# kabachuha/sd-webui-text2video

Hardware: NVIDIA H100
Metric: denoised frames/sec (UNet+VAE) ModelScope 24fx256^2 50-step (higher is better)
Workload: dtype f16 (fp32 accumulate / norms / softmax)

## Files before the change

### sd-webui-text2video_b200/csrc/elementwise.cu

```cuda
#include "common.cuh"
#include "kernels.cuh"

#include <math_constants.h>

namespace t2v {

namespace {

inline int grid_for(long long n, int threads, int cap = 132 * 16) {
    long long b = (n + threads - 1) / threads;
    if (b > cap) b = cap;
    if (b < 1) b = 1;
    return static_cast<int>(b);
}
#define GRID_STRIDE(i, n) \
    for (long long i = blockIdx.x * static_cast<long long>(blockDim.x) + threadIdx.x; i < (n); \
         i += static_cast<long long>(gridDim.x) * blockDim.x)

__global__ void ingest_kernel(const void* x, int x_is_f32, __half* tok, long long ld, int cpad, int C, int F, int h, int w,
                              long long frame0, long long nframes, float scale) {
    const long long P = static_cast<long long>(h) * w;
    const long long rows = nframes * P;
    GRID_STRIDE(i, rows * cpad) {
        const long long r = i / cpad;
        const int c = static_cast<int>(i - r * cpad);
        float v = 0.f;
        if (c < C) {
            const long long p = r % P;
            const long long bf = frame0 + r / P;
            const int f = static_cast<int>(bf % F);
            const int b = static_cast<int>(bf / F);
            const long long src = ((static_cast<long long>(b) * C + c) * F + f) * P + p;
            v = x_is_f32 ? reinterpret_cast<const float*>(x)[src] : __half2float(reinterpret_cast<const __half*>(x)[src]);
            v *= scale;
        }
        tok[r * ld + c] = __float2half_rn(v);
    }
}

__global__ void egress_kernel(const __half* tok, long long ld, void* out, int out_is_f32, int B, int C, int F, int h,
                              int w) {
    const long long P = static_cast<long long>(h) * w;
    const long long n = static_cast<long long>(B) * C * F * P;
    GRID_STRIDE(i, n) {
        const long long p = i % P;
        long long t = i / P;
        const int f = static_cast<int>(t % F);
        t /= F;
        const int c = static_cast<int>(t % C);
        const int b = static_cast<int>(t / C);
        const __half v = tok[((static_cast<long long>(b) * F + f) * P + p) * ld + c];
        if (out_is_f32) reinterpret_cast<float*>(out)[i] = __half2float(v);
        else reinterpret_cast<__half*>(out)[i] = v;
    }
}

__global__ void upsample2x_kernel(const uint4* x, uint4* y, long long nframes, int h, int w, int C8) {
    const int H = 2 * h, W = 2 * w;
    const long long n = nframes * H * W * C8;
    GRID_STRIDE(i, n) {
        const int c = static_cast<int>(i % C8);
        long long t = i / C8;
        const int X = static_cast<int>(t % W);
        t /= W;
        const int Y = static_cast<int>(t % H);
        const long long f = t / H;
        y[i] = __ldg(x + ((f * h + (Y >> 1)) * w + (X >> 1)) * C8 + c);
    }
}

__global__ void im2col_s2_kernel(const uint4* x, uint4* col, long long nframes, int h, int w, int C8, int pad_lo) {
    const int ho = pad_lo ? (h + 1) / 2 : h / 2, wo = pad_lo ? (w + 1) / 2 : w / 2;
    const long long n = nframes * ho * wo * 9 * C8;
    GRID_STRIDE(i, n) {
        const int c = static_cast<int>(i % C8);
        long long t = i / C8;
        const int tap = static_cast<int>(t % 9);
        t /= 9;
        const int xo = static_cast<int>(t % wo);
        t /= wo;
        const int yo = static_cast<int>(t % ho);
        const long long f = t / ho;
        const int yi = 2 * yo + tap / 3 - pad_lo;
        const int xi = 2 * xo + tap % 3 - pad_lo;
        uint4 v = make_uint4(0, 0, 0, 0);
        if (yi >= 0 && yi < h && xi >= 0 && xi < w) v = __ldg(x + ((f * h + yi) * w + xi) * C8 + c);
        col[i] = v;
    }
}

__global__ void concat_kernel(const __half* a, long long lda, int Ca8, const __half* b, long long ldb, int Cb8,
                              __half* out, long long ldo, long long rows) {
    const int T8 = Ca8 + Cb8;
    GRID_STRIDE(i, rows * T8) {
        const long long r = i / T8;
        const int c = static_cast<int>(i - r * T8);
        uint4 v;
        if (c < Ca8) v = __ldg(reinterpret_cast<const uint4*>(a + r * lda) + c);
        else v = __ldg(reinterpret_cast<const uint4*>(b + r * ldb) + (c - Ca8));
        reinterpret_cast<uint4*>(out + r * ldo)[c] = v;
    }
}

__global__ void time_sinusoid_kernel(const float* t, __half* out, int B, int dim) {
    const int half_dim = dim / 2;
    GRID_STRIDE(i, static_cast<long long>(B) * dim) {
        const int b = static_cast<int>(i / dim);
        const int j = static_cast<int>(i % dim);
        float v = 0.f;
        if (j < 2 * half_dim) {
            const int k = j < half_dim ? j : j - half_dim;
            const float freq = powf(10000.0f, -(static_cast<float>(k) / static_cast<float>(half_dim)));
            const float s = t[b] * freq;
            v = j < half_dim ? cosf(s) : sinf(s);
        }
        out[i] = __float2half_rn(v);
    }
}

__global__ void __launch_bounds__(256) small_linear_kernel(const __half* x, long long ldx, const __half* W,
                                                           const __half* bias, const __half* addend, __half* y,
                                                           long long ldy, int B, int N, int K, int silu_in) {
    const int lane = threadIdx.x & 31;
    const int n = blockIdx.x * (blockDim.x >> 5) + (threadIdx.x >> 5);
    if (n >= N) return;
    const __half* wr = W + static_cast<long long>(n) * K;
    for (int b = 0; b < B; ++b) {
        float acc = 0.f;
        for (int k = lane * 8; k < K; k += 256) {
            const uint4 wv = __ldg(reinterpret_cast<const uint4*>(wr + k));
            const uint4 xv = __ldg(reinterpret_cast<const uint4*>(x + b * ldx + k));
            const __half* wh = reinterpret_cast<const __half*>(&wv);
            const __half* xh = reinterpret_cast<const __half*>(&xv);
#pragma unroll
            for (int e = 0; e < 8; ++e) {
                float xe = __half2float(xh[e]);
                if (silu_in) xe = __half2float(__float2half_rn(xe / (1.0f + __expf(-xe))));
                acc += xe * __half2float(wh[e]);
            }
        }
#pragma unroll
        for (int o = 16; o > 0; o >>= 1) acc += __shfl_xor_sync(0xffffffffu, acc, o);
        if (lane == 0) {
            if (bias) acc += __half2float(bias[n]);
            float r = __half2float(__float2half_rn(acc));
            if (addend) r += __half2float(addend[n]);
            y[b * ldy + n] = __float2half_rn(r);
        }
    }
}

__global__ void __launch_bounds__(256) softmax_rows_kernel(const __half* x, __half* y, long long rows, int cols,
                                                           float scale) {
    const int lane = threadIdx.x & 31;
    const long long row = blockIdx.x * static_cast<long long>(blockDim.x >> 5) + (threadIdx.x >> 5);
    if (row >= rows) return;
    const __half* xr = x + row * cols;
    float m = -CUDART_INF_F;
    for (int c = lane; c < cols; c += 32) m = fmaxf(m, __half2float(__float2half_rn(__half2float(xr[c]) * scale)));
#pragma unroll
    for (int o = 16; o > 0; o >>= 1) m = fmaxf(m, __shfl_xor_sync(0xffffffffu, m, o));
    float s = 0.f;
    for (int c = lane; c < cols; c += 32) s += __expf(__half2float(__float2half_rn(__half2float(xr[c]) * scale)) - m);
#pragma unroll
    for (int o = 16; o > 0; o >>= 1) s += __shfl_xor_sync(0xffffffffu, s, o);
    const float inv = 1.0f / s;
    __half* yr = y + row * cols;
    for (int c = lane; c < cols; c += 32)
        yr[c] = __float2half_rn(__expf(__half2float(__float2half_rn(__half2float(xr[c]) * scale)) - m) * inv);
}

__global__ void transpose_kernel(const __half* x, __half* y, int R, int C) {
    __shared__ __half tile[32][34];
    const long long base = static_cast<long long>(blockIdx.z) * R * C;
    const int c0 = blockIdx.x * 32, r0 = blockIdx.y * 32;
    for (int j = threadIdx.y; j < 32; j += 8) {
        const int r = r0 + j, c = c0 + threadIdx.x;
        if (r < R && c < C) tile[j][threadIdx.x] = x[base + static_cast<long long>(r) * C + c];
    }
    __syncthreads();
    for (int j = threadIdx.y; j < 32; j += 8) {
        const int c = c0 + j, r = r0 + threadIdx.x;
        if (r < R && c < C) y[base + static_cast<long long>(c) * R + r] = tile[threadIdx.x][j];
    }
}

__global__ void frames_to_u8_kernel(const __half* tok, long long ld, uint8_t* out, long long pixels) {
    GRID_STRIDE(i, pixels * 3) {
        const long long p = i / 3;
        const int c = static_cast<int>(i - p * 3);
        float v = __half2float(tok[p * ld + c]);
        v = __fadd_rn(__fmul_rn(v, 0.5f), 0.5f);
        v = fminf(fmaxf(v, 0.f), 1.f);
        out[i] = static_cast<uint8_t>(__fmul_rn(v, 255.0f));
    }
}

__global__ void pixel_unshuffle_kernel(const void* x, int x_is_f32, __half* tok, int N, int Cc, int H, int W) {
    const int h8 = H / 8, w8 = W / 8;
    const int groups = Cc * 8;
    const long long n = static_cast<long long>(N) * h8 * w8 * groups;
    GRID_STRIDE(i, n) {
        const int g = static_cast<int>(i % groups);
        long long t = i / groups;
        const int xo = static_cast<int>(t % w8);
        t /= w8;
        const int yo = static_cast<int>(t % h8);
        const long long f = t / h8;
        const int c = g >> 3, ky = g & 7;
        const long long src = ((f * Cc + c) * H + (8 * yo + ky)) * static_cast<long long>(W) + 8 * xo;
        uint4 o;
        __half* oh = reinterpret_cast<__half*>(&o);
#pragma unroll
        for (int j = 0; j < 8; ++j)
            oh[j] = x_is_f32 ? __float2half_rn(reinterpret_cast<const float*>(x)[src + j]) : reinterpret_cast<const __half*>(x)[src + j];
        reinterpret_cast<uint4*>(tok)[i] = o;
    }
}

__global__ void relu_kernel(uint4* x, long long n8) {
    const __half2 z = __float2half2_rn(0.f);
    GRID_STRIDE(i, n8) {
        uint4 v = x[i];
        __half2* h = reinterpret_cast<__half2*>(&v);
#pragma unroll
        for (int k = 0; k < 4; ++k) h[k] = __hmax2_nan(h[k], z);
        x[i] = v;
    }
}

__global__ void avgpool2x2_kernel(const uint4* x, uint4* y, long long nframes, int h, int w, int C8) {
    const int ho = h / 2, wo = w / 2;
    GRID_STRIDE(i, nframes * ho * wo * C8) {
        const int c = static_cast<int>(i % C8);
        long long t = i / C8;
        const int xo = static_cast<int>(t % wo);
        t /= wo;
        const int yo = static_cast<int>(t % ho);
        const long long f = t / ho;
        float acc[8] = {0.f, 0.f, 0.f, 0.f, 0.f, 0.f, 0.f, 0.f};
#pragma unroll
        for (int tap = 0; tap < 4; ++tap) {
            const uint4 v = __ldg(x + ((f * h + 2 * yo + (tap >> 1)) * w + 2 * xo + (tap & 1)) * C8 + c);
            const __half2* hv = reinterpret_cast<const __half2*>(&v);
#pragma unroll
            for (int k = 0; k < 4; ++k) {
                const float2 a = __half22float2(hv[k]);
                acc[2 * k] += a.x;
                acc[2 * k + 1] += a.y;
            }
        }
        uint4 o;
        __half2* oh = reinterpret_cast<__half2*>(&o);
#pragma unroll
        for (int k = 0; k < 4; ++k) oh[k] = __floats2half2_rn(acc[2 * k] * 0.25f, acc[2 * k + 1] * 0.25f);
        y[i] = o;
    }
}

__global__ void feature_add_kernel(__half* x, long long ldx, const __half* f, int C8, long long rows, long long rows_per_sample,
                                   int f_samples) {
    GRID_STRIDE(i, rows * C8) {
        const long long r = i / C8;
        const int c = static_cast<int>(i - r * C8);
        const long long s = r / rows_per_sample;
        const long long fr = (s % f_samples) * rows_per_sample + (r - s * rows_per_sample);
        uint4* xp = reinterpret_cast<uint4*>(x + r * ldx) + c;
        uint4 a = *xp;
        const uint4 b = __ldg(reinterpret_cast<const uint4*>(f + fr * (static_cast<long long>(C8) * 8)) + c);
        __half2* ah = reinterpret_cast<__half2*>(&a);
        const __half2* bh = reinterpret_cast<const __half2*>(&b);
#pragma unroll
        for (int k = 0; k < 4; ++k) {
            const float2 u = __half22float2(ah[k]), v = __half22float2(bh[k]);
            ah[k] = __floats2half2_rn(u.x + v.x, u.y + v.y);
        }
        *xp = a;
    }
}

__global__ void frames_to_f32_kernel(const __half* tok, long long ld, float* out, int n, int H, int W) {
    const long long P = static_cast<long long>(H) * W;
    GRID_STRIDE(i, static_cast<long long>(n) * 3 * P) {
        const long long p = i % P;
        const long long t = i / P;
        const int c = static_cast<int>(t % 3);
        const long long f = t / 3;
        out[i] = __half2float(tok[(f * P + p) * ld + c]);
    }
}

__global__ void pack_conv_kernel(const void* src, int src_is_f32, __half* dst, int Cout, int Cin, int taps, int n_alloc,
// ... 201 lines not shown
        out[i] = __dadd_rn(__dmul_rn(a, __dsub_rn(1.0, m)), __dmul_rn(noise[i], m));
        if (mask != nullptr) mask[i] = m;
    }
}

__global__ void q_sample_blend_kernel(QSampleBlendParams p) {
    const long long hw = static_cast<long long>(p.shape[3]) * p.shape[4];
    const long long n = static_cast<long long>(p.shape[0]) * p.shape[1] * p.shape[2] * hw;
    GRID_STRIDE(i, n) {
        const int x = static_cast<int>(i % p.shape[4]);
        long long r = i / p.shape[4];
        const int y = static_cast<int>(r % p.shape[3]);
        r /= p.shape[3];
        const int t = static_cast<int>(r % p.shape[2]);
        r /= p.shape[2];
        const int c = static_cast<int>(r % p.shape[1]);
        const int b = static_cast<int>(r / p.shape[1]);
        const int idx[5] = {b, c, t, y, x};
        long long ox = 0, on = 0, om = 0;
#pragma unroll
        for (int d = 0; d < 5; ++d) {
            ox += idx[d] * p.x0_stride[d];
            on += idx[d] * p.noise_stride[d];
            om += idx[d] * p.mask_stride[d];
        }
        const float known = __fadd_rn(__fmul_rn(p.a[b], p.x0[ox]), __fmul_rn(p.s[b], p.noise[on]));
        if (p.mask == nullptr) {
            p.out[i] = known;
        } else {
            const float m = p.mask[om];
            p.out[i] = __fadd_rn(__fmul_rn(known, m), __fmul_rn(__fsub_rn(1.0f, m), p.img[i]));
        }
    }
}

__global__ void lora_merge_kernel(__half* __restrict__ w, const __half* __restrict__ A, const __half* __restrict__ B, int out, int cols,
                                  int rank, float alpha, int temporal_mean) {
    const long long n = static_cast<long long>(out) * cols;
    const int a_cols = temporal_mean ? cols * 3 : cols;
    GRID_STRIDE(i, n) {
        const int o = static_cast<int>(i / cols);
        const int j = static_cast<int>(i - static_cast<long long>(o) * cols);
        float d;
        if (temporal_mean) {
            float sum = 0.f;
            for (int q = 0; q < 3; ++q) {
                float acc = 0.f;
                for (int r = 0; r < rank; ++r)
                    acc = fmaf(__half2float(B[static_cast<long long>(o) * rank + r]), __half2float(A[static_cast<long long>(r) * a_cols + j * 3 + q]), acc);
                sum += __half2float(__float2half_rn(acc));
            }
            d = __half2float(__float2half_rn(sum / 3.0f));
        } else {
            float acc = 0.f;
            for (int r = 0; r < rank; ++r)
                acc = fmaf(__half2float(B[static_cast<long long>(o) * rank + r]), __half2float(A[static_cast<long long>(r) * a_cols + j]), acc);
            d = __half2float(__float2half_rn(acc));
        }
        const float scaled = __half2float(__float2half_rn(d * alpha));
        w[i] = __float2half_rn(__half2float(w[i]) + scaled);
    }
}

__device__ __forceinline__ float widen(float v) { return v; }
__device__ __forceinline__ float widen(__half v) { return __half2float(v); }

template <class T>
__global__ void lora_apply_kernel(__half* __restrict__ w, const T* __restrict__ up, const T* __restrict__ down, int out, int cols,
                                  int rank, float alpha) {
    const long long n = static_cast<long long>(out) * cols;
    GRID_STRIDE(i, n) {
        const int o = static_cast<int>(i / cols);
        const int j = static_cast<int>(i - static_cast<long long>(o) * cols);
        float acc = 0.f;
        for (int r = 0; r < rank; ++r)
            acc = fmaf(widen(up[static_cast<long long>(o) * rank + r]), widen(down[static_cast<long long>(r) * cols + j]), acc);
        w[i] = __float2half_rn(__fadd_rn(__half2float(w[i]), __fmul_rn(alpha, acc)));
    }
}

inline int ok() { return launch_status("elementwise launch"); }

}

int ingest_latent(const void* x, int x_is_f32, __half* tok, long long ld, int cpad, int B, int C, int F, int h, int w,
                  float scale, cudaStream_t stream) {
    return ingest_latent_frames(x, x_is_f32, tok, ld, cpad, C, F, h, w, 0, static_cast<long long>(B) * F, scale, stream);
}
int ingest_latent_frames(const void* x, int x_is_f32, __half* tok, long long ld, int cpad, int C, int F, int h, int w,
                         long long frame0, long long nframes, float scale, cudaStream_t stream) {
    const long long n = nframes * h * w * cpad;
    ingest_kernel<<<grid_for(n, 256), 256, 0, stream>>>(x, x_is_f32, tok, ld, cpad, C, F, h, w, frame0, nframes, scale);
    return ok();
}
int egress_latent(const __half* tok, long long ld, void* out, int out_is_f32, int B, int C, int F, int h, int w,
                  cudaStream_t stream) {
    const long long n = static_cast<long long>(B) * C * F * h * w;
    egress_kernel<<<grid_for(n, 256), 256, 0, stream>>>(tok, ld, out, out_is_f32, B, C, F, h, w);
    return ok();
}
int upsample2x(const __half* x, __half* y, int nframes, int h, int w, int C, cudaStream_t stream) {
    if (C % 8) return -1;
    const long long n = static_cast<long long>(nframes) * 4 * h * w * (C / 8);
    upsample2x_kernel<<<grid_for(n, 256), 256, 0, stream>>>(reinterpret_cast<const uint4*>(x), reinterpret_cast<uint4*>(y),
                                                            nframes, h, w, C / 8);
    return ok();
}
int im2col_s2(const __half* x, __half* col, int nframes, int h, int w, int C, cudaStream_t stream, int pad_lo) {
    if (C % 8) return -1;
    const long long n = static_cast<long long>(nframes) * ((pad_lo ? (h + 1) / 2 : h / 2)) * ((pad_lo ? (w + 1) / 2 : w / 2)) * 9 * (C / 8);
    im2col_s2_kernel<<<grid_for(n, 256), 256, 0, stream>>>(reinterpret_cast<const uint4*>(x), reinterpret_cast<uint4*>(col),
                                                           nframes, h, w, C / 8, pad_lo);
    return ok();
}
int pixel_unshuffle_ingest(const void* x, int x_is_f32, __half* tok, int N, int Cc, int H, int W, cudaStream_t stream) {
    if (H % 8 || W % 8) return -1;
    const long long n = static_cast<long long>(N) * (H / 8) * (W / 8) * Cc * 8;
    pixel_unshuffle_kernel<<<grid_for(n, 256), 256, 0, stream>>>(x, x_is_f32, tok, N, Cc, H, W);
    return ok();
}
int relu_inplace(__half* x, long long rows, int C, cudaStream_t stream) {
    if (C % 8) return -1;
    const long long n8 = rows * (C / 8);
    relu_kernel<<<grid_for(n8, 256), 256, 0, stream>>>(reinterpret_cast<uint4*>(x), n8);
    return ok();
}
int avgpool2x2(const __half* x, __half* y, int nframes, int h, int w, int C, cudaStream_t stream) {
    if (C % 8) return -1;
    const long long n = static_cast<long long>(nframes) * (h / 2) * (w / 2) * (C / 8);
    avgpool2x2_kernel<<<grid_for(n, 256), 256, 0, stream>>>(reinterpret_cast<const uint4*>(x), reinterpret_cast<uint4*>(y),
                                                            nframes, h, w, C / 8);
    return ok();
}
int feature_add(__half* x, long long ldx, const __half* f, int C, long long rows, long long rows_per_sample, int f_samples,
                cudaStream_t stream) {
    if (C % 8 || ldx % 8 || rows_per_sample < 1 || f_samples < 1) return -1;
    const long long n = rows * (C / 8);
    feature_add_kernel<<<grid_for(n, 256), 256, 0, stream>>>(x, ldx, f, C / 8, rows, rows_per_sample, f_samples);
    return ok();
}
int concat_cols(const __half* a, long long lda, int Ca, const __half* b, long long ldb, int Cb, __half* out,
                long long ldo, long long rows, cudaStream_t stream) {
    if ((Ca % 8) || (Cb % 8) || (lda % 8) || (ldb % 8) || (ldo % 8)) return -1;
    const long long n = rows * ((Ca + Cb) / 8);
    concat_kernel<<<grid_for(n, 256), 256, 0, stream>>>(a, lda, Ca / 8, b, ldb, Cb / 8, out, ldo, rows);
    return ok();
}
int time_sinusoid(const float* t, __half* out, int B, int dim, cudaStream_t stream) {
    time_sinusoid_kernel<<<grid_for(static_cast<long long>(B) * dim, 256), 256, 0, stream>>>(t, out, B, dim);
    return ok();
}
int small_linear(const __half* x, long long ldx, const __half* W, const __half* bias, const __half* addend, __half* y,
                 long long ldy, int B, int N, int K, int silu_in, cudaStream_t stream) {
    if ((K % 8) || (ldx % 8)) return -1;
    small_linear_kernel<<<(N + 7) / 8, 256, 0, stream>>>(x, ldx, W, bias, addend, y, ldy, B, N, K, silu_in);
    return ok();
}
int softmax_rows(const __half* x, __half* y, long long rows, int cols, float scale, cudaStream_t stream) {
    softmax_rows_kernel<<<static_cast<unsigned int>((rows + 7) / 8), 256, 0, stream>>>(x, y, rows, cols, scale);
    return ok();
}
int transpose_batched(const __half* x, __half* y, int nb, int R, int C, cudaStream_t stream) {
    dim3 grid((C + 31) / 32, (R + 31) / 32, nb);
    transpose_kernel<<<grid, dim3(32, 8), 0, stream>>>(x, y, R, C);
    return ok();
}
int frames_to_u8(const __half* tok, long long ld, uint8_t* out, long long pixels, cudaStream_t stream) {
    frames_to_u8_kernel<<<grid_for(pixels * 3, 256), 256, 0, stream>>>(tok, ld, out, pixels);
    return ok();
}
int frames_to_f32_nchw(const __half* tok, long long ld, float* out, int n, int H, int W, cudaStream_t stream) {
    frames_to_f32_kernel<<<grid_for(static_cast<long long>(n) * 3 * H * W, 256), 256, 0, stream>>>(tok, ld, out, n, H, W);
    return ok();
}
int pack_conv_weight(const void* src, int src_is_f32, __half* dst, int Cout, int Cin, int taps, int n_alloc, int k_alloc,
                     cudaStream_t stream) {
    const long long n = static_cast<long long>(taps) * n_alloc * k_alloc;
    pack_conv_kernel<<<grid_for(n, 256), 256, 0, stream>>>(src, src_is_f32, dst, Cout, Cin, taps, n_alloc, k_alloc);
    return ok();
}
int pack_geglu_weight(const void* w, const void* b, int src_is_f32, __half* wdst, __half* bdst, int H, int K, int bn,
                      cudaStream_t stream) {
    if ((2 * H) % bn) return -1;
    pack_geglu_kernel<<<grid_for(static_cast<long long>(2) * H * K, 256), 256, 0, stream>>>(w, b, src_is_f32, wdst, bdst, H, K, bn);
    return ok();
}
int splitk_reduce(const float* part, int splits, long long split_stride, long long rows, int N, const __half* bias,
                  int bias_rows, long long bias_stride, const __half* residual, long long ldr, __half* out, long long ldo,
                  cudaStream_t stream) {
    if ((N & 7) || (ldo & 7) || (residual && (ldr & 7)) || (bias && (bias_stride & 7))) return -1;
    splitk_reduce_kernel<<<grid_for(rows * (N / 8), 256), 256, 0, stream>>>(part, splits, split_stride, rows, N / 8, bias,
                                                                            bias_rows, bias_stride, residual, ldr, out, ldo);
    return ok();
}
int fold_ln_into_linear(const __half* w, const __half* bias, const __half* gamma, const __half* beta, __half* wout,
                        float* colsum, float* bias32, int N, int K, cudaStream_t stream) {
    fold_ln_kernel<<<(N + 7) / 8, 256, 0, stream>>>(w, bias, gamma, beta, wout, colsum, bias32, N, K);
    return ok();
}
int convert_to_f16(const void* src, int src_is_f32, __half* dst, long long n, cudaStream_t stream) {
    convert_kernel<<<grid_for(n, 256), 256, 0, stream>>>(src, src_is_f32, dst, n);
    return ok();
}
int ddim_step(const DdimStepParams& p, cudaStream_t stream) {
    ddim_step_kernel<<<grid_for(p.n, 256), 256, 0, stream>>>(p);
    return ok();
}
int ddim_threshold_step(const DdimStepParams& p, int B, float percentile, float* s, void* ws, cudaStream_t stream) {
    if (percentile > 0.f) {
        ddim_x0_kernel<<<grid_for(p.n, 256), 256, 0, stream>>>(p);
        int rc = ok();
        if (rc != 0) return rc;
        if ((rc = abs_quantile(p.x_out, B, p.n / B, percentile, s, ws, stream)) != 0) return rc;
    }
    ddim_threshold_kernel<<<grid_for(p.n, 256), 256, 0, stream>>>(p, percentile > 0.f ? s : nullptr, p.n / B);
    return ok();
}
int lincomb(float* out, const float* const* src, const float* coef, int n_src, long long n, cudaStream_t stream) {
    if (n_src < 1 || n_src > 8) return -1;
    LincombArgs a;
    for (int i = 0; i < n_src; ++i) {
        a.src[i] = src[i];
        a.coef[i] = coef[i];
    }
    a.n_src = n_src;
    lincomb_kernel<<<grid_for(n, 256), 256, 0, stream>>>(out, a, n);
    return ok();
}
int lora_merge_weight(__half* w, const __half* A, const __half* B, int out, int cols, int rank, float alpha, int temporal_mean,
                      cudaStream_t stream) {
    const long long n = static_cast<long long>(out) * cols;
    lora_merge_kernel<<<grid_for(n, 256), 256, 0, stream>>>(w, A, B, out, cols, rank, alpha, temporal_mean);
    return ok();
}
int lora_apply_weight(__half* w, const void* up, const void* down, int dtype, int out, int cols, int rank, float alpha,
                      cudaStream_t stream) {
    const long long n = static_cast<long long>(out) * cols;
    if (dtype == 1)
        lora_apply_kernel<float><<<grid_for(n, 256), 256, 0, stream>>>(w, static_cast<const float*>(up),
                                                                       static_cast<const float*>(down), out, cols, rank, alpha);
    else
        lora_apply_kernel<__half><<<grid_for(n, 256), 256, 0, stream>>>(w, static_cast<const __half*>(up),
                                                                        static_cast<const __half*>(down), out, cols, rank, alpha);
    return ok();
}

int latent_blend(const float* img, int img_frames, const double* noise, const double* w, double* out, double* mask, int BC, int F,
                 long long hw, cudaStream_t stream) {
    const long long n = static_cast<long long>(BC) * F * hw;
    latent_blend_kernel<<<grid_for(n, 256), 256, 0, stream>>>(img, img_frames, noise, w, out, mask, n, F, hw);
    return ok();
}

int q_sample_blend(const QSampleBlendParams& p, cudaStream_t stream) {
    const long long n = static_cast<long long>(p.shape[0]) * p.shape[1] * p.shape[2] * p.shape[3] * p.shape[4];
    q_sample_blend_kernel<<<grid_for(n, 256), 256, 0, stream>>>(p);
    return ok();
}

int cfg_x0(const float* x, const void* eps_c, const void* eps_u, int eps_is_f32, float* x0, long long n, float g,
           float alpha, float sigma, int cfg_fp16, cudaStream_t stream) {
    cfg_x0_kernel<<<grid_for(n, 256), 256, 0, stream>>>(x, eps_c, eps_u, eps_is_f32, x0, n, g, alpha, sigma, cfg_fp16);
    return ok();
}

}
```

### sd-webui-text2video_b200/csrc/unet.cu

```cuda
#include "../../include/t2v_b200.h"
#include "runtime.cuh"

#include <algorithm>
#include <cmath>
#include <cstdlib>
#include <cstdio>
#include <cstring>
#include <memory>

namespace t2v {

namespace {

struct Blk {
    enum Kind { STEM, RES, ST, TT, DOWN, UP, STT } kind;
    std::string prefix;
    int cin = 0, cout = 0, heads = 0, inner = 0;
};

constexpr int kMaxFeat = 8;

struct IO {
    __half* x_tok;
    float* t;
// ... 180 lines not shown
                lin(p + ".proj_in", b.inner, b.cin);
                tblock(p + ".transformer_blocks.0", b.inner, c.context_dim);
                lin(p + ".proj_out", b.cin, b.inner);
                break;
            case Blk::TT:
                norm(p + ".norm", b.cin);
                P.expect(p + ".proj_in.weight", {b.inner, b.cin, 1});
                P.expect(p + ".proj_in.bias", {b.inner});
                tblock(p + ".transformer_blocks.0", b.inner, b.inner);
                P.expect(p + ".proj_out.weight", {b.cin, b.inner, 1});
                P.expect(p + ".proj_out.bias", {b.cin});
                break;
            case Blk::DOWN:
                P.expect(p + ".op.weight", {b.cout, b.cin, 3, 3});
                P.expect(p + ".op.bias", {b.cout});
                break;
            case Blk::UP:
                P.expect(p + ".conv.weight", {b.cout, b.cin, 3, 3});
                P.expect(p + ".conv.bias", {b.cout});
                break;
        }
    }
    norm("out.0", c.dim);
    P.expect("out.2.weight", {c.out_dim, c.dim, 3, 3});
    P.expect("out.2.bias", {c.out_dim});
}


void enumerate_vc(t2v_unet* u) {
    const t2v_unet_config& c = u->cfg;
    const int mc = c.dim, nm = c.n_mult;
    auto name = [](const char* base, int n, int k) {
        char buf[64];
        snprintf(buf, sizeof(buf), "%s.%d.%d", base, n, k);
        return std::string(buf);
    };
    u->ins.push_back({Blk{Blk::STEM, "input_blocks.0.0", c.in_dim, mc, 0, 0}});
    std::vector<int> chans{mc};
    int ch = mc;
    float scale = 1.0f;
    for (int level = 0; level < nm; ++level) {
        for (int j = 0; j < c.num_res_blocks; ++j) {
            const int n = static_cast<int>(u->ins.size());
            std::vector<Blk> blk;
            blk.push_back(Blk{Blk::RES, name("input_blocks", n, 0), ch, mc * c.dim_mult[level], 0, 0});
            ch = mc * c.dim_mult[level];
            if (in_scales(c, scale)) blk.push_back(Blk{Blk::STT, name("input_blocks", n, 1), ch, ch, c.num_heads, ch});
            u->ins.push_back(blk);
            chans.push_back(ch);
        }
        if (level != nm - 1) {
            const int n = static_cast<int>(u->ins.size());
            u->ins.push_back({Blk{Blk::DOWN, name("input_blocks", n, 0), ch, ch, 0, 0}});
            chans.push_back(ch);
            scale /= 2.0f;
        }
    }
    u->mid = {Blk{Blk::RES, "middle_block.0", ch, ch, 0, 0}, Blk{Blk::STT, "middle_block.1", ch, ch, c.num_heads, ch},
              Blk{Blk::RES, "middle_block.2", ch, ch, 0, 0}};
    for (int level = nm - 1; level >= 0; --level) {
        for (int i = 0; i < c.num_res_blocks + 1; ++i) {
            const int n = static_cast<int>(u->outs.size());
            const int ich = chans.back();
            chans.pop_back();
            std::vector<Blk> blk;
            blk.push_back(Blk{Blk::RES, name("output_blocks", n, 0), ch + ich, mc * c.dim_mult[level], 0, 0});
            ch = mc * c.dim_mult[level];
            if (in_scales(c, scale))
                blk.push_back(Blk{Blk::STT, name("output_blocks", n, static_cast<int>(blk.size())), ch, ch, c.num_heads, ch});
            if (level != 0 && i == c.num_res_blocks) {
                blk.push_back(Blk{Blk::UP, name("output_blocks", n, static_cast<int>(blk.size())), ch, ch, 0, 0});
                scale *= 2.0f;
            }
            u->outs.push_back(blk);
        }
    }
}

void expect_params_vc(t2v_unet* u) {
    ParamStore& P = u->params;
    const t2v_unet_config& c = u->cfg;
    const int E = c.dim * 4;
    auto lin = [&](const std::string& p, int o, int i, bool bias = true) {
        P.expect(p + ".weight", {o, i});
        if (bias) P.expect(p + ".bias", {o});
    };
    auto norm = [&](const std::string& p, int ch) {
        P.expect(p + ".weight", {ch});
        P.expect(p + ".bias", {ch});
    };
    auto conv = [&](const std::string& p, int o, int i, int k) {
        P.expect(p + ".weight", {o, i, 1, k, k});
        P.expect(p + ".bias", {o});
    };
    lin("time_embed.0", E, c.dim);
    lin("time_embed.2", E, E);
    std::vector<Blk> all;
    for (auto& b : u->ins) all.insert(all.end(), b.begin(), b.end());
    all.insert(all.end(), u->mid.begin(), u->mid.end());
    for (auto& b : u->outs) all.insert(all.end(), b.begin(), b.end());
    for (const Blk& b : all) {
        const std::string& p = b.prefix;
        switch (b.kind) {
            case Blk::STEM: conv(p, b.cout, b.cin, 3); break;
            case Blk::RES:
                norm(p + ".in_layers.0", b.cin);
                conv(p + ".in_layers.2", b.cout, b.cin, 3);
                lin(p + ".emb_layers.1", b.cout, E);
                norm(p + ".out_layers.0", b.cout);
                conv(p + ".out_layers.3", b.cout, b.cout, 3);
                if (b.cin != b.cout) conv(p + ".skip_connection", b.cout, b.cin, 1);
                break;
            case Blk::STT: {
                const int inner = b.inner, d = inner / b.heads;
                norm(p + ".norm", b.cin);
                conv(p + ".proj_in", inner, b.cin, 1);
                conv(p + ".proj_out", b.cin, inner, 1);
                const std::string t = p + ".transformer_blocks.0";
                const char* att[4] = {"attn1", "attn2", "attn1_tmp", "attn2_tmp"};
                for (int a = 0; a < 4; ++a) {
                    const std::string ap = t + "." + att[a];
                    const int kd = a == 1 ? c.context_dim : inner;
                    lin(ap + ".to_q", inner, inner, false);
                    lin(ap + ".to_k", inner, kd, false);
                    lin(ap + ".to_v", inner, kd, false);
                    lin(ap + ".to_out.0", inner, inner);
                    if (a >= 2) {
                        P.expect(ap + ".relative_position_k.embeddings_table", {2 * c.temporal_length + 1, d});
                        P.expect(ap + ".relative_position_v.embeddings_table", {2 * c.temporal_length + 1, d});
                    }
                }
                lin(t + ".ff.net.0.proj", inner * 8, inner);
                lin(t + ".ff.net.2", inner, inner * 4);
                for (int n = 1; n <= 5; ++n) norm(t + ".norm" + std::to_string(n), inner);
                break;
            }
            case Blk::DOWN: conv(p + ".op", b.cout, b.cin, 3); break;
            case Blk::UP: conv(p + ".conv", b.cout, b.cin, 3); break;
            default: break;
        }
    }
    norm("out.0", c.dim);
    conv("out.2", c.out_dim, c.dim, 3);
}

struct Ctx : NetCtx {
    t2v_unet* u;
    int B, F, h, w, L;
    int Bc;
    int Fl;
    int rank, nranks;
    char* slab;
    __half* emb;
    __half* ctx;
    Plan* plan;
};

int own_pixels(const Ctx& c, int hcur, int wcur) {
    if (c.nranks <= 1) return hcur * wcur;
    int pb[SHARD_MAX_RANKS + 1];
    shard_partition(hcur * wcur, c.nranks, pb);
    return pb[c.rank + 1] - pb[c.rank];
}

Tok exchange(Ctx& c, const Tok& x, bool to_ps, int hcur, int wcur) {
    const int P = hcur * wcur;
    const int np = own_pixels(c, hcur, wcur);
    const long long rows = to_ps ? static_cast<long long>(c.B) * c.F * np : static_cast<long long>(c.B) * c.Fl * P;
    Tok y = c.b->alloc(rows, x.C);
    PlanShard* ps = c.plan_shard;
    const int k = ps->n_xchg++;
    if (k >= SHARD_MAX_XCHG - 1) {
        set_error("frame-sharded plan: more than %d layout exchanges", SHARD_MAX_XCHG - 1);
        c.b->error = -31;
        return y;
    }
    if (!c.b->dry()) ps->dst_off[k] = reinterpret_cast<char*>(y.p) - c.slab;
    XchgParams xp;
    memset(&xp, 0, sizeof(xp));
    xp.slot = k;
    xp.to_ps = to_ps ? 1 : 0;
    xp.B = c.B; xp.F = c.F; xp.P = P; xp.C = x.C;
    xp.ld_src = x.ld; xp.ld_dst = y.ld;
    xp.src = x.p;
    for (int r = 0; r <= c.nranks; ++r) xp.fb[r] = ps->fb[r];
    shard_partition(P, c.nranks, xp.pb);
    const ShardPeers* peers = c.shard_peers;
    const int me = c.rank, nr = c.nranks, sms = c.b->sms();
    __half* own = y.p;
    char lab[96];
    snprintf(lab, sizeof(lab), "exchange %s rows=%lld C=%d", to_ps ? "FS->PS" : "PS->FS", rows, x.C);
    c.b->step([=](cudaStream_t s) {
        if (!ps->connected) return -40;
        XchgParams q = xp;
        q.peers = *peers;
        for (int r = 0; r < nr; ++r)
            q.dst[r] = r == me ? own : reinterpret_cast<__half*>(ps->peer_slab[r] + ps->peer_dst_off[r][k]);
        return shard_exchange(q, sms, s);
    }, 1, STEP_OTHER, 0.0, lab);
    return y;
}

void tap(Ctx& c, const std::string& name, const Tok& t, int h, int w) {
    if (c.u->taps_enabled && !c.b->dry()) c.plan->taps[name] = {t, {h, w}};
}

long long norm_rows(const Ctx& c, long long P) { return c.u->cfg.arch == 1 ? P * c.F : P; }


AttnParams attn_params(const Tok& o, int heads) {
    AttnParams a;
    memset(&a, 0, sizeof(a));
    a.o = o.p;
    a.heads = heads;
    a.head_dim = o.C / heads;
    a.scale = 1.0f / std::sqrt(static_cast<float>(a.head_dim));
    a.kv_batch_div = 1;
    a.b_inner = 1;
    return a;
}

void attn_step(Ctx& c, const AttnParams& a, const char* label) {
    c.b->step([a](cudaStream_t s) { return attention(a, s); }, 1, STEP_ATTN,
              4.0 * a.batch * a.heads * static_cast<double>(a.sq) * a.skv * a.head_dim, label);
}

Tok qkv_proj(Ctx& c, const Tok& x, const std::string& ap, const std::string& lnp) {
    const __half* w = w_cat(c, {ap + ".to_q.weight", ap + ".to_k.weight", ap + ".to_v.weight"});
    return ln_linear(c, x, lnp, ap + ".qkv", w, nullptr, 3 * x.C, nullptr);
}

Tok attn_out(Ctx& c, const Tok& x, const Tok& o, const Tok& in, const std::string& ap) {
    c.b->free(in);
    Tok y = linear(c, o, prm(c, ap + ".to_out.0.weight"), x.C, prm(c, ap + ".to_out.0.bias"), &x);
    c.b->free(o);
    c.b->free(x);
    return y;
}

Tok attn_spatial(Ctx& c, const Tok& x, const std::string& ap, const std::string& lnp, int heads, long long P, const char* label) {
    const int C = x.C;
    Tok o = c.b->alloc(x.rows, C);
    Tok qkv = qkv_proj(c, x, ap, lnp);
    AttnParams a = attn_params(o, heads);
    a.q = qkv.p;
    a.k = qkv.p + C;
    a.v = qkv.p + 2 * C;
    a.batch = static_cast<int>(x.rows / P);
    a.sq = a.skv = static_cast<int>(P);
    a.q_bs = a.k_bs = a.v_bs = P * qkv.ld;
    a.q_ss = a.k_ss = a.v_ss = qkv.ld;
    a.o_bs = P * o.ld;
    a.o_ss = o.ld;
    attn_step(c, a, label);
    return attn_out(c, x, o, qkv, ap);
}

Tok attn_cross(Ctx& c, const Tok& x, const std::string& ap, const std::string& lnp, int heads, long long P, const char* label) {
    const int C = x.C;
    Tok o = c.b->alloc(x.rows, C);
    Tok q = ln_linear(c, x, lnp, ap + ".to_q", prm(c, ap + ".to_q.weight"), nullptr, C, nullptr);
    Tok ctx_tok;
    ctx_tok.p = c.ctx;
    ctx_tok.rows = static_cast<long long>(c.Bc) * c.L;
    ctx_tok.C = c.u->cfg.context_dim;
    ctx_tok.ld = ctx_tok.C;
    const __half* wkv = w_cat(c, {ap + ".to_k.weight", ap + ".to_v.weight"});
    Tok kv = linear(c, ctx_tok, wkv, 2 * C, nullptr, nullptr);
    AttnParams a = attn_params(o, heads);
    a.q = q.p;
    a.k = kv.p;
    a.v = kv.p + C;
    a.batch = static_cast<int>(x.rows / P);
    a.sq = static_cast<int>(P);
    a.skv = c.L;
    a.q_bs = P * q.ld;
    a.q_ss = q.ld;
    a.k_bs = a.v_bs = static_cast<long long>(c.L) * kv.ld;
    a.k_ss = a.v_ss = kv.ld;
    a.kv_batch_div = c.Fl * (c.B / c.Bc);
    a.o_bs = P * o.ld;
    a.o_ss = o.ld;
    attn_step(c, a, label);
    c.b->free(kv);
    return attn_out(c, x, o, q, ap);
}

Tok attn_temporal(Ctx& c, const Tok& x, const std::string& ap, const std::string& lnp, int heads, long long P) {
    const int C = x.C;
    Tok o = c.b->alloc(x.rows, C);
    Tok qkv = qkv_proj(c, x, ap, lnp);
    AttnParams a = attn_params(o, heads);
    a.q = qkv.p;
    a.k = qkv.p + C;
    a.v = qkv.p + 2 * C;
    a.batch = static_cast<int>(c.B * P);
    a.b_inner = static_cast<int>(P);
    a.sq = a.skv = c.F;
    a.q_bs = a.k_bs = a.v_bs = static_cast<long long>(c.F) * P * qkv.ld;
    a.q_bsi = a.k_bsi = a.v_bsi = qkv.ld;
    a.q_ss = a.k_ss = a.v_ss = P * qkv.ld;
    a.o_bs = static_cast<long long>(c.F) * P * o.ld;
    a.o_bsi = o.ld;
    a.o_ss = P * o.ld;
    attn_step(c, a, "attn temporal");
    return attn_out(c, x, o, qkv, ap);
}

Tok attn_relpos(Ctx& c, const Tok& x, const std::string& ap, const std::string& lnp, int heads, long long P) {
    const int C = x.C, d = C / heads;
    Tok o = c.b->alloc(x.rows, C);
    Tok qkv = qkv_proj(c, x, ap, lnp);
    RelposParams r;
    memset(&r, 0, sizeof(r));
    r.q = qkv.p;
    r.k = qkv.p + C;
    r.v = qkv.p + 2 * C;
    r.o = o.p;
    r.table_k = prm(c, ap + ".relative_position_k.embeddings_table");
    r.table_v = prm(c, ap + ".relative_position_v.embeddings_table");
    r.n_seq = static_cast<long long>(c.B) * P;
    r.seq_inner = P;
    r.bs_outer = static_cast<long long>(c.F) * P * qkv.ld;
    r.bs_inner = qkv.ld;
    r.ss = P * qkv.ld;
    r.o_bs_outer = static_cast<long long>(c.F) * P * o.ld;
    r.o_bs_inner = o.ld;
    r.o_ss = P * o.ld;
    r.heads = heads;
    r.head_dim = d;
    r.T = c.F;
    r.max_rel = c.u->cfg.temporal_length;
    r.scale = 1.0f / std::sqrt(static_cast<float>(d));
    const int nrel = 2 * r.max_rel + 1;
    c.b->step([r](cudaStream_t s) { return attention_relpos(r, s); }, 1, STEP_ATTN,
              4.0 * r.n_seq * heads * static_cast<double>(c.F) * (c.F + nrel) * d, "attn temporal relpos (vc)");
    return attn_out(c, x, o, qkv, ap);
}

Tok feed_forward(Ctx& c, const Tok& x, const std::string& p) {
    const int C = x.C, H = 4 * C;
    const int bn = (2 * H) % 256 == 0 ? 256 : ((2 * H) % 128 == 0 ? 128 : 64);
    Geglu g = w_geglu(c, p + ".ff.net.0.proj", H, C, bn);
    Tok gg = ln_linear(c, x, p + ".norm3", p + ".ff.net.0.proj#geglu" + std::to_string(bn), g.w, g.b, 2 * H, nullptr, GEMM_GEGLU, bn);
    Tok y = linear(c, gg, prm(c, p + ".ff.net.2.weight"), C, prm(c, p + ".ff.net.2.bias"), &x);
    c.b->free(gg);
    c.b->free(x);
    return y;
}

Tok transformer(Ctx& c, const Tok& x, const Blk& blk, int hcur, int wcur) {
    const bool temporal = blk.kind == Blk::TT;
    const long long Pfull = static_cast<long long>(hcur) * wcur;
    const long long P = temporal ? own_pixels(c, hcur, wcur) : Pfull;
    const std::string& p = blk.prefix;
    Tok n = group_norm(c, x, p + ".norm", temporal ? P * c.F : norm_rows(c, P), 1e-6f, false,
                       (temporal && c.nranks > 1) ? Pfull * c.F : 0);
    Tok h = linear(c, n, prm(c, p + ".proj_in.weight"), blk.inner, prm(c, p + ".proj_in.bias"), nullptr);
    c.b->free(n);
    const std::string t = p + ".transformer_blocks.0";
    const int heads = blk.heads;
    switch (blk.kind) {
        case Blk::ST:
            h = attn_spatial(c, h, t + ".attn1", t + ".norm1", heads, P, "attn spatial");
            h = attn_cross(c, h, t + ".attn2", t + ".norm2", heads, P, "attn cross");
            break;
        case Blk::TT:
            h = attn_temporal(c, h, t + ".attn1", t + ".norm1", heads, P);
            h = attn_temporal(c, h, t + ".attn2", t + ".norm2", heads, P);
            break;
        default:
            h = attn_spatial(c, h, t + ".attn1", t + ".norm1", heads, P, "attn spatial (vc)");
            h = attn_relpos(c, h, t + ".attn1_tmp", t + ".norm4", heads, P);
            h = attn_cross(c, h, t + ".attn2", t + ".norm2", heads, P, "attn cross (vc)");
            h = attn_relpos(c, h, t + ".attn2_tmp", t + ".norm5", heads, P);
            break;
    }
    h = feed_forward(c, h, t);
    Tok y = linear(c, h, prm(c, p + ".proj_out.weight"), blk.cin, prm(c, p + ".proj_out.bias"), &x);
    c.b->free(h);
    return y;
}

Tok res_block(Ctx& c, const Tok& x, const Blk& blk, int hcur, int wcur) {
    const std::string& p = blk.prefix;
    const long long P = static_cast<long long>(hcur) * wcur;
    const int Co = blk.cout;
    const int E = c.u->cfg.dim * 4;
    __half* bias1 = reinterpret_cast<__half*>(c.b->alloc_bytes(static_cast<size_t>(c.B) * Co * sizeof(__half)));
    {
        const __half* we = prm(c, p + ".emb_layers.1.weight");
        const __half* be = prm(c, p + ".emb_layers.1.bias");
        const __half* bc = prm(c, p + ".in_layers.2.bias");
        const __half* emb = c.emb;
        const int B = c.B;
        c.b->step([=](cudaStream_t s) { return small_linear(emb, E, we, be, bc, bias1, Co, B, Co, E, 1, s); });
    }
    Tok a = group_norm(c, x, p + ".in_layers.0", norm_rows(c, P), 1e-5f, true);
    Tok h = conv3x3(c, a, p + ".in_layers.2.weight", bias1, static_cast<int>(c.Fl * P), Co, Co, hcur, wcur, nullptr);
    c.b->free(a);
    Tok bn_ = group_norm(c, h, p + ".out_layers.0", norm_rows(c, P), 1e-5f, true);
    c.b->free(h);
    Tok skip = x;
    bool own_skip = false;
    if (blk.cin != blk.cout) {
        skip = linear(c, x, prm(c, p + ".skip_connection.weight"), Co, prm(c, p + ".skip_connection.bias"), nullptr);
        own_skip = true;
    }
    Tok h2 = conv3x3(c, bn_, p + ".out_layers.3.weight", prm(c, p + ".out_layers.3.bias"), 0, 0, Co, hcur, wcur, &skip);
    c.b->free(bn_);
    if (own_skip) c.b->free(skip);
    c.b->free_bytes(bias1);
    if (c.u->cfg.arch == 1) return h2;
    const long long Pt = own_pixels(c, hcur, wcur);
    if (c.nranks > 1) {
        Tok hp = exchange(c, h2, true, hcur, wcur);
        c.b->free(h2);
        h2 = hp;
    }
    const long long Rt = h2.rows;
    const char* names[4] = {"conv1", "conv2", "conv3", "conv4"};
    const int idx[4] = {2, 3, 3, 3};
    Tok y = h2;
    for (int i = 0; i < 4; ++i) {
        const std::string tp = p + ".temopral_conv." + names[i];
        Tok g = group_norm(c, y, tp + ".0", Pt * c.F, 1e-5f, true, c.nranks > 1 ? P * c.F : 0);
        const std::string wn = tp + "." + std::to_string(idx[i]);
        const __half* w = w_conv(c, wn + ".weight", 3);
        Tok y2 = c.b->alloc(Rt, Co);
        GemmProblem pr = base_problem(g, Co, w, Co, Co, y2);
        pr.nd = 3;
        pr.dim[0] = static_cast<int>(Pt);
        pr.dim[1] = c.F;
        pr.dim[2] = c.B;
        taps_temporal(pr);
        pr.bias = prm(c, wn + ".bias");
        if (i == 3) {
            pr.residual = h2.p;
            pr.ldr = h2.ld;
        }
        c.b->gemm(pr);
        c.b->free(g);
        if (i > 0) c.b->free(y);
        y = y2;
    }
    c.b->free(h2);
    return y;
}

Tok downsample(Ctx& c, const Tok& x, const Blk& blk, int hcur, int wcur) {
    const int frames = static_cast<int>(x.rows / (static_cast<long long>(hcur) * wcur));
    const int ho = (hcur + 1) / 2, wo = (wcur + 1) / 2;
    Tok col = c.b->alloc(static_cast<long long>(frames) * ho * wo, 9 * x.C);
    const Tok xx = x;
    c.b->step([=](cudaStream_t s) { return im2col_s2(xx.p, col.p, frames, hcur, wcur, xx.C, s); });
    const __half* w = w_conv_kmajor(c, blk.prefix + ".op.weight");
    Tok y = linear(c, col, w, blk.cout, prm(c, blk.prefix + ".op.bias"), nullptr);
    c.b->free(col);
    return y;
}

Tok upsample(Ctx& c, const Tok& x, const Blk& blk, int hcur, int wcur) {
    const int frames = static_cast<int>(x.rows / (static_cast<long long>(hcur) * wcur));
    Tok u = c.b->alloc(x.rows * 4, x.C);
    const Tok xx = x;
    c.b->step([=](cudaStream_t s) { return upsample2x(xx.p, u.p, frames, hcur, wcur, xx.C, s); });
    Tok y = conv3x3(c, u, blk.prefix + ".conv.weight", prm(c, blk.prefix + ".conv.bias"), 0, 0, blk.cout, 2 * hcur,
                    2 * wcur, nullptr);
    c.b->free(u);
    return y;
}

bool feature_block(int id) { return (id + 1) % 3 == 0; }
int n_feature_blocks(const t2v_unet* u) {
    int n = 0;
    for (size_t id = 0; id < u->ins.size(); ++id) n += feature_block(static_cast<int>(id)) ? 1 : 0;
    return n;
}

int build(t2v_unet* u, Plan* plan, Arena* arena, bool dry, cudaStream_t stream, int B, int Bc, int F, int h, int w, int L,
          IO* io, int feats_B = 0) {
    Builder bld(plan, arena, dry, num_sms());
    Ctx c;
    c.params = &u->params;
    c.b = &bld;
    c.stream = stream;
    c.gn_ws = u->gn_ws.ptr;
    c.u = u;
    c.B = B; c.Bc = Bc; c.F = F; c.h = h; c.w = w; c.L = L;
    c.emb = nullptr; c.ctx = nullptr; c.plan = plan;
    c.Fl = F; c.rank = 0; c.nranks = 1; c.slab = plan->slab;
    const bool sharded = u->shard_on && plan->shard != nullptr;
    if (sharded) {
        c.rank = u->peers.rank;
        c.nranks = u->peers.nranks;
        c.Fl = plan->shard->fb[c.rank + 1] - plan->shard->fb[c.rank];
        c.shard_peers = &u->peers;
        c.plan_shard = plan->shard.get();
        plan->shard->n_xchg = 0;
        plan->shard->n_gn = 0;
        if (!dry) {
            ShardComm* comm = u->comm;
            bld.step([comm](cudaStream_t s) { return shard_bump_epoch(comm, s); }, 1, STEP_OTHER, 0.0, "epoch");
        }
    }
    const t2v_unet_config& cfg = u->cfg;
    const int E = cfg.dim * 4;
    const long long R0 = static_cast<long long>(B) * c.Fl * h * w;
    const int cin_pad = round_up(cfg.in_dim, 8);

    Tok x0 = bld.alloc(R0, cin_pad);
    io->x_tok = x0.p;
    io->t = reinterpret_cast<float*>(bld.alloc_bytes(static_cast<size_t>(B) * sizeof(float)));
    Tok ctx_tok = bld.alloc(static_cast<long long>(Bc) * L, cfg.context_dim);
    c.ctx = ctx_tok.p;
    io->ctx = ctx_tok.p;
    io->n_feat = 0;
    if (feats_B > 0) {
        int hf = h, wf = w;
        for (size_t id = 0; id < u->ins.size(); ++id) {
            const Blk& b0 = u->ins[id][0];
            if (b0.kind == Blk::DOWN) {
                hf = (hf + 1) / 2;
                wf = (wf + 1) / 2;
            }
            if (!feature_block(static_cast<int>(id))) continue;
            if (io->n_feat >= kMaxFeat) {
                set_error("more than %d adapter injection points", kMaxFeat);
                return -7;
            }
            const int Cf = u->ins[id].back().cout;
            Tok f = bld.alloc(static_cast<long long>(feats_B) * F * hf * wf, Cf);
            io->feat[io->n_feat] = f.p;
            io->feat_elems[io->n_feat] = f.rows * f.C;
            io->n_feat += 1;
        }
    }
    __half* sinus = reinterpret_cast<__half*>(bld.alloc_bytes(static_cast<size_t>(B) * cfg.dim * sizeof(__half)));
    __half* e1 = reinterpret_cast<__half*>(bld.alloc_bytes(static_cast<size_t>(B) * E * sizeof(__half)));
    __half* e2 = reinterpret_cast<__half*>(bld.alloc_bytes(static_cast<size_t>(B) * E * sizeof(__half)));
    c.emb = e2;
    {
        const float* tp = io->t;
        const int dim = cfg.dim;
        const __half* w0 = prm(c, "time_embed.0.weight");
        const __half* b0 = prm(c, "time_embed.0.bias");
        const __half* w2 = prm(c, "time_embed.2.weight");
        const __half* b2 = prm(c, "time_embed.2.bias");
        bld.step([=](cudaStream_t s) { return time_sinusoid(tp, sinus, B, dim, s); });
        bld.step([=](cudaStream_t s) { return small_linear(sinus, dim, w0, b0, nullptr, e1, E, B, E, dim, 0, s); });
        bld.step([=](cudaStream_t s) { return small_linear(e1, E, w2, b2, nullptr, e2, E, B, E, E, 1, s); });
    }

    int hc = h, wc = w;
    std::vector<Tok> xs;
    std::vector<std::pair<int, int>> xs_hw;
    Tok x = x0;
    bool x_is_io = true;
    bool x_ps = false;
    auto release = [&](const Tok& t) {
        for (const Tok& s : xs)
            if (s.p == t.p) return;
        if (t.p == x0.p && x_is_io) return;
        bld.free(t);
    };
    auto to_layout = [&](bool want_ps) {
        if (!sharded || x_ps == want_ps) return;
        Tok y = exchange(c, x, want_ps, hc, wc);
        release(x);
        x_is_io = false;
        x = y;
        x_ps = want_ps;
    };
    auto run_block = [&](const std::vector<Blk>& blk) {
        for (const Blk& b : blk) {
            Tok y;
            to_layout(b.kind == Blk::TT);
            switch (b.kind) {
                case Blk::STEM:
                    y = conv3x3(c, x, b.prefix + ".weight", prm(c, b.prefix + ".bias"), 0, 0, b.cout, hc, wc, nullptr);
                    break;
                case Blk::RES: y = res_block(c, x, b, hc, wc); break;
                case Blk::ST:
                case Blk::TT:
                case Blk::STT: y = transformer(c, x, b, hc, wc); break;
                case Blk::DOWN:
                    y = downsample(c, x, b, hc, wc);
                    hc = (hc + 1) / 2;
                    wc = (wc + 1) / 2;
                    break;
                case Blk::UP:
                    y = upsample(c, x, b, hc, wc);
                    hc *= 2;
                    wc *= 2;
                    break;
            }
            if (sharded && b.kind == Blk::RES) x_ps = true;
            if (sharded && x_ps) tap(c, b.prefix, y, 1, own_pixels(c, hc, wc));
            else tap(c, b.prefix, y, hc, wc);
            release(x);
            x_is_io = false;
            x = y;
        }
    };
    int feat_i = 0;
    for (size_t id = 0; id < u->ins.size(); ++id) {
        run_block(u->ins[id]);
        to_layout(false);
        if (feats_B > 0 && feature_block(static_cast<int>(id))) {
            const Tok xx = x;
            const __half* f = io->feat[feat_i++];
            const long long per_sample = static_cast<long long>(F) * hc * wc;
            const int fb = feats_B;
            bld.step([=](cudaStream_t s) { return feature_add(xx.p, xx.ld, f, xx.C, xx.rows, per_sample, fb, s); }, 1, STEP_OTHER,
                     0.0, "adapter feature add");
        }
        xs.push_back(x);
        xs_hw.push_back({hc, wc});
    }
    run_block(u->mid);
    for (auto& blk : u->outs) {
        to_layout(false);
        Tok skip = xs.back();
        xs.pop_back();
        xs_hw.pop_back();
        Tok cat = bld.alloc(x.rows, x.C + skip.C);
        {
            const Tok xa = x, sb = skip;
            bld.step([=](cudaStream_t s) {
                return concat_cols(xa.p, xa.ld, xa.C, sb.p, sb.ld, sb.C, cat.p, cat.ld, xa.rows, s);
            });
        }
        bool x_on_stack = false;
        for (const Tok& s : xs)
            if (s.p == x.p) x_on_stack = true;
        if (!x_on_stack && x.p != skip.p) bld.free(x);
        bld.free(skip);
        x = cat;
        run_block(blk);
    }
    to_layout(false);
    Tok g = group_norm(c, x, "out.0", norm_rows(c, static_cast<long long>(hc) * wc), 1e-5f, true);
    bld.free(x);
    Tok o = conv3x3(c, g, "out.2.weight", prm(c, "out.2.bias"), 0, 0, cfg.out_dim, hc, wc, nullptr, 16);
    bld.free(g);
    io->out_tok = o.p;
    tap(c, "out", o, hc, wc);
    return bld.error;
}

std::string plan_key(const t2v_unet* u, int B, int Bc, int F, int h, int w, int L, int feats_B) {
    char key[128];
    snprintf(key, sizeof(key), "%d,%d,%d,%d,%d,%d,%d/%d", B, F, h, w, L, u->taps_enabled ? 1 : 0, u->shard_on ? u->peers.rank : 0,
             u->shard_on ? u->peers.nranks : 1);
    if (feats_B > 0) {
        const size_t n = strlen(key);
        snprintf(key + n, sizeof(key) - n, ",a%d", feats_B);
    }
    if (Bc != B) {
        const size_t n = strlen(key);
        snprintf(key + n, sizeof(key) - n, ",c%d", Bc);
    }
    return key;
}

std::shared_ptr<PlanShard> new_plan_shard(const t2v_unet* u, int F) {
    if (!u->shard_on) return nullptr;
    std::shared_ptr<PlanShard> s(new PlanShard());
    s->own_rank = u->peers.rank;
    shard_partition(F, u->peers.nranks, s->fb);
    return s;
}

PlanCache<IO>::Entry* get_plan(t2v_unet* u, int B, int Bc, int F, int h, int w, int L, cudaStream_t stream, int feats_B = 0) {
    const std::string key = plan_key(u, B, Bc, F, h, w, L, feats_B);
    if (auto* e = u->plans.find(key, u->params.version())) return e;
    if (!u->params.complete("UNet")) return nullptr;
    size_t need = std::max(gn_workspace_bytes(F * h * w, B, num_sms()), gn_workspace_bytes(h * w, B * F, num_sms()));
    need = std::max(need, gn_workspace_bytes(1, B * F, num_sms()));
    if (u->gn_ws.ensure(need + (1 << 20), stream)) u->plans.clear(stream);
    if (!u->gn_ws.ptr) return nullptr;
    if (u->shard_on) {
        if (u->cfg.arch != 0) {
            set_error("frame sharding is built for the ModelScope UNetSD (arch 0)");
            return nullptr;
        }
        int deepest = h * w;
        for (int i = 1; i < u->cfg.n_mult; ++i) deepest = ((h + (1 << i) - 1) >> i) * ((w + (1 << i) - 1) >> i);
        if (F < u->peers.nranks || deepest < u->peers.nranks || B > SHARD_MAX_INST) {
            set_error("frame sharding over %d ranks needs >= %d frames, >= %d pixels at the deepest level (got %d) and B <= %d",
                      u->peers.nranks, u->peers.nranks, u->peers.nranks, deepest, SHARD_MAX_INST);
            return nullptr;
        }
    }
    std::unique_ptr<Plan> shell(new Plan());
    shell->shard = new_plan_shard(u, F);
    return u->plans.build(key, u->params.version(), stream, std::move(shell),
                          u->taps_enabled || getenv("T2V_ARENA_NO_REUSE") != nullptr, "UNet",
                          [&](Plan* p, Arena* a, bool dry, IO* io) { return build(u, p, a, dry, stream, B, Bc, F, h, w, L, io, feats_B); });
}

const std::pair<Tok, std::pair<int, int>>* find_tap(t2v_unet* u, const char* name) {
    auto* entry = u->plans.latest();
    if (entry) {
        auto it = entry->plan->taps.find(name);
// ... 375 lines not shown
```

Before: 12.50.

## Batch all ResBlock time-embedding projections into one small_linear launch

Concatenates the emb_layers weights, biases and conv biases of every ResBlock and computes all per-block time-embedding biases in a single small_linear call at the start, instead of one launch per ResBlock. Each block's conv then reads its bias from a column slice of that shared buffer, with a larger leading dimension. The small_linear kernel now stages the SiLU-activated input row in shared memory once per block rather than recomputing SiLU per warp per element. This cuts kernel-launch count and redundant exp work, but it keeps a buffer alive across the whole UNet and limits K to 16384.

```diff
diff --git a/sd-webui-text2video_b200/csrc/elementwise.cu b/sd-webui-text2video_b200/csrc/elementwise.cu
--- a/sd-webui-text2video_b200/csrc/elementwise.cu
+++ b/sd-webui-text2video_b200/csrc/elementwise.cu
@@ -121,23 +121,27 @@
 __global__ void __launch_bounds__(256) small_linear_kernel(const __half* x, long long ldx, const __half* W,
                                                            const __half* bias, const __half* addend, __half* y,
                                                            long long ldy, int B, int N, int K, int silu_in) {
+    extern __shared__ __align__(16) __half xs[];
     const int lane = threadIdx.x & 31;
     const int n = blockIdx.x * (blockDim.x >> 5) + (threadIdx.x >> 5);
-    if (n >= N) return;
     const __half* wr = W + static_cast<long long>(n) * K;
     for (int b = 0; b < B; ++b) {
+        __syncthreads();
+        for (int k = threadIdx.x; k < K; k += blockDim.x) {
+            float xe = __half2float(x[b * ldx + k]);
+            if (silu_in) xe = __half2float(__float2half_rn(xe / (1.0f + __expf(-xe))));
+            xs[k] = __float2half_rn(xe);
+        }
+        __syncthreads();
+        if (n >= N) continue;
         float acc = 0.f;
         for (int k = lane * 8; k < K; k += 256) {
             const uint4 wv = __ldg(reinterpret_cast<const uint4*>(wr + k));
-            const uint4 xv = __ldg(reinterpret_cast<const uint4*>(x + b * ldx + k));
+            const uint4 xv = *reinterpret_cast<const uint4*>(xs + k);
             const __half* wh = reinterpret_cast<const __half*>(&wv);
             const __half* xh = reinterpret_cast<const __half*>(&xv);
 #pragma unroll
-            for (int e = 0; e < 8; ++e) {
-                float xe = __half2float(xh[e]);
-                if (silu_in) xe = __half2float(__float2half_rn(xe / (1.0f + __expf(-xe))));
-                acc += xe * __half2float(wh[e]);
-            }
+            for (int e = 0; e < 8; ++e) acc += __half2float(xh[e]) * __half2float(wh[e]);
         }
 #pragma unroll
         for (int o = 16; o > 0; o >>= 1) acc += __shfl_xor_sync(0xffffffffu, acc, o);
@@ -645,8 +649,9 @@
 }
 int small_linear(const __half* x, long long ldx, const __half* W, const __half* bias, const __half* addend, __half* y,
                  long long ldy, int B, int N, int K, int silu_in, cudaStream_t stream) {
-    if ((K % 8) || (ldx % 8)) return -1;
-    small_linear_kernel<<<(N + 7) / 8, 256, 0, stream>>>(x, ldx, W, bias, addend, y, ldy, B, N, K, silu_in);
+    if ((K % 8) || (ldx % 8) || K > 16384) return -1;
+    small_linear_kernel<<<(N + 7) / 8, 256, static_cast<size_t>(K) * sizeof(__half), stream>>>(x, ldx, W, bias, addend, y, ldy, B,
+                                                                                            N, K, silu_in);
     return ok();
 }
 int softmax_rows(const __half* x, __half* y, long long rows, int cols, float scale, cudaStream_t stream) {
diff --git a/sd-webui-text2video_b200/csrc/unet.cu b/sd-webui-text2video_b200/csrc/unet.cu
--- a/sd-webui-text2video_b200/csrc/unet.cu
+++ b/sd-webui-text2video_b200/csrc/unet.cu
@@ -356,6 +356,9 @@
     int rank, nranks;
     char* slab;
     __half* emb;
+    __half* emb_bias;
+    long long emb_bias_ld;
+    std::map<std::string, long long> emb_bias_col;
     __half* ctx;
     Plan* plan;
 };
@@ -586,22 +589,43 @@
     return y;
 }
 
+void emb_bias_rows(Ctx& c, int E) {
+    std::vector<std::string> we, be, bc;
+    long long n = 0;
+    auto add = [&](const Blk& b) {
+        c.emb_bias_col[b.prefix] = n;
+        n += b.cout;
+        we.push_back(b.prefix + ".emb_layers.1.weight");
+        be.push_back(b.prefix + ".emb_layers.1.bias");
+        bc.push_back(b.prefix + ".in_layers.2.bias");
+    };
+    for (const std::vector<Blk>& blk : c.u->ins)
+        for (const Blk& b : blk)
+            if (b.kind == Blk::RES) add(b);
+    for (const Blk& b : c.u->mid)
+        if (b.kind == Blk::RES) add(b);
+    for (const std::vector<Blk>& blk : c.u->outs)
+        for (const Blk& b : blk)
+            if (b.kind == Blk::RES) add(b);
+    c.emb_bias_ld = n;
+    c.emb_bias = reinterpret_cast<__half*>(c.b->alloc_bytes(static_cast<size_t>(c.B) * n * sizeof(__half)));
+    const __half* w = w_cat(c, we);
+    const __half* bias = w_cat(c, be);
+    const __half* addend = w_cat(c, bc);
+    const __half* emb = c.emb;
+    __half* y = c.emb_bias;
+    const int B = c.B;
+    const int N = static_cast<int>(n);
+    c.b->step([=](cudaStream_t s) { return small_linear(emb, E, w, bias, addend, y, N, B, N, E, 1, s); });
+}
+
 Tok res_block(Ctx& c, const Tok& x, const Blk& blk, int hcur, int wcur) {
     const std::string& p = blk.prefix;
     const long long P = static_cast<long long>(hcur) * wcur;
     const int Co = blk.cout;
-    const int E = c.u->cfg.dim * 4;
-    __half* bias1 = reinterpret_cast<__half*>(c.b->alloc_bytes(static_cast<size_t>(c.B) * Co * sizeof(__half)));
-    {
-        const __half* we = prm(c, p + ".emb_layers.1.weight");
-        const __half* be = prm(c, p + ".emb_layers.1.bias");
-        const __half* bc = prm(c, p + ".in_layers.2.bias");
-        const __half* emb = c.emb;
-        const int B = c.B;
-        c.b->step([=](cudaStream_t s) { return small_linear(emb, E, we, be, bc, bias1, Co, B, Co, E, 1, s); });
-    }
+    const __half* bias1 = c.emb_bias + c.emb_bias_col.at(p);
     Tok a = group_norm(c, x, p + ".in_layers.0", norm_rows(c, P), 1e-5f, true);
-    Tok h = conv3x3(c, a, p + ".in_layers.2.weight", bias1, static_cast<int>(c.Fl * P), Co, Co, hcur, wcur, nullptr);
+    Tok h = conv3x3(c, a, p + ".in_layers.2.weight", bias1, static_cast<int>(c.Fl * P), c.emb_bias_ld, Co, hcur, wcur, nullptr);
     c.b->free(a);
     Tok bn_ = group_norm(c, h, p + ".out_layers.0", norm_rows(c, P), 1e-5f, true);
     c.b->free(h);
@@ -614,7 +638,6 @@
     Tok h2 = conv3x3(c, bn_, p + ".out_layers.3.weight", prm(c, p + ".out_layers.3.bias"), 0, 0, Co, hcur, wcur, &skip);
     c.b->free(bn_);
     if (own_skip) c.b->free(skip);
-    c.b->free_bytes(bias1);
     if (c.u->cfg.arch == 1) return h2;
     const long long Pt = own_pixels(c, hcur, wcur);
     if (c.nranks > 1) {
@@ -755,6 +778,7 @@
         bld.step([=](cudaStream_t s) { return small_linear(sinus, dim, w0, b0, nullptr, e1, E, B, E, dim, 0, s); });
         bld.step([=](cudaStream_t s) { return small_linear(e1, E, w2, b2, nullptr, e2, E, B, E, E, 1, s); });
     }
+    emb_bias_rows(c, E);
 
     int hc = h, wc = w;
     std::vector<Tok> xs;
```

Measured after the change: 12.54 (median of 6 runs). No clear change (+0.4%).
